# diogoneiss/kubernetes-machine-learning-server

Measured on AMD Instinct MI355X. Metric: itemsets/sec mined (FP-Growth, every frequent itemset of every size + its support, one dataset split over the GPUs), higher is better.
Workload: dtype uint64 tid-bitmaps / exact integer supports

## Files before the change

csrc/emu/kmls/wave.hpp:

```cpp
#pragma once

#include <hip/hip_runtime.h>

#define KMLS_DYN_LDS(T, name) T* name = (T*)emu::dyn_lds()

namespace kmls {
namespace kern {

inline unsigned vzero() { return 0u; }

template <typename T>
using gptr = T*;
template <typename T>
inline gptr<T> as_global(T* p) { return p; }
template <typename T>
inline gptr<T> as_global_addr(unsigned long long a) { return (T*)a; }

inline unsigned long long bcast64(unsigned long long v, int src) {
  return emu::xchg(v, src);
}
inline unsigned long long shfl_xor64(unsigned long long v, int m) {
  return emu::xchg(v, emu::tl->lane ^ m);
}
inline unsigned uni(unsigned v) { return (unsigned)__builtin_amdgcn_readfirstlane((int)v); }
inline unsigned lane0(unsigned v) { return (unsigned)emu::xchg((unsigned long long)v, 0); }
inline unsigned long long lane0_64(unsigned long long v) { return emu::xchg(v, 0); }
inline unsigned long long uni64(unsigned long long v) {
  return ((unsigned long long)uni((unsigned)(v >> 32)) << 32) | uni((unsigned)v);
}

inline unsigned long long ld_agent(const unsigned long long* p) { return __atomic_load_n(p, __ATOMIC_SEQ_CST); }
inline unsigned ld_agent(const unsigned* p) { return __atomic_load_n(p, __ATOMIC_SEQ_CST); }
inline void st_agent(unsigned long long* p, unsigned long long v) { __atomic_store_n(p, v, __ATOMIC_SEQ_CST); }
inline void st_agent(unsigned* p, unsigned v) { __atomic_store_n(p, v, __ATOMIC_SEQ_CST); }
inline void wait_stores() { __atomic_thread_fence(__ATOMIC_SEQ_CST); }
inline void wait_short(unsigned) { std::this_thread::yield(); }

}
}
```

csrc/host/bindings_gpu.cpp:

```cpp
#include <cstring>
#include <pybind11/numpy.h>
#include <pybind11/pybind11.h>
#include <pybind11/stl.h>

#include "../kernels/kernels.hpp"
#include "kmls/gpu.hpp"
#include "kmls/trace.hpp"

namespace py = pybind11;

namespace kmls {

namespace {
template <typename T>
py::array_t<T> to_array(std::vector<T>&& v) {
  auto* heap = new std::vector<T>(std::move(v));
  py::capsule owner(heap, [](void* p) { delete reinterpret_cast<std::vector<T>*>(p); });
  return py::array_t<T>({(py::ssize_t)heap->size()}, {(py::ssize_t)sizeof(T)}, heap->data(), owner);
}

template <typename T>
py::array_t<T> pinned_array(const std::shared_ptr<void>& buf, int64_t n) {
  if (!buf) return py::array_t<T>(0);
  auto* keep = new std::shared_ptr<void>(buf);
// ... 467 lines not shown
        o.assign = assign;
        o.trace = trace;
        o.presplit_cost = presplit_cost;
        o.presplit_budget = presplit_budget;
        o.steal = steal;
        o.steal_idle = steal_idle;
        o.budget0 = budget0;
        o.budget = budget;
        o.split_min = split_min;
        o.blocks_per_cu = blocks_per_cu;
        o.stack_mb = stack_mb;
        gpu::Comm* c = comm.is_none() ? nullptr : comm.cast<gpu::Comm*>();
        gpu::DeepResult r;
        {
          py::gil_scoped_release nogil;
          r = g.mine_deep(ms, max_len, rank, world, c, o);
        }
        py::dict d;
        d["per_level"] = r.per_level;
        d["n_itemsets"] = r.n_itemsets;
        d["n_frequent_items"] = r.n_frequent_items;
        d["max_depth"] = r.max_depth;
        d["candidates"] = r.candidates;
        d["chunks"] = r.chunks;
        d["level2_tasks"] = r.level2_tasks;
        char buf[64];
        std::snprintf(buf, sizeof buf, "%016llx%016llx", (unsigned long long)r.digest_sum,
                      (unsigned long long)r.digest_xor);
        d["digest"] = std::string(buf);
        d["round_tasks"] = r.round_tasks;
        d["spilled_tasks"] = r.spilled_tasks;
        d["handoffs"] = r.handoffs;
        d["leaf_candidates"] = r.leaf_candidates;
        d["leaf_m_default"] = gpu::kDeepLeafDefault;
        d["leaf_m_max"] = kern::deep_leaf_max();
        d["round_ms"] = r.round_ms;
        py::dict ph;
        ph["prologue"] = r.ms_prologue;
        ph["level2_classes"] = r.ms_root;
        ph["rounds"] = r.ms_rounds;
        ph["combine"] = r.ms_combine;
        ph["total"] = r.ms_total;
        ph["assign"] = r.ms_assign;
        ph["presplit"] = r.ms_presplit;
        d["presplit"] = py::make_tuple(r.presplit_in, r.presplit_out);
        if (emit) {
          d["arena_nodes"] = r.arena_nodes;
          d["arena_cap"] = r.arena_cap;
        }
        d["phases_ms"] = ph;
        if (trace) {
          const size_t nw = r.trace.size() / kern::kDeepTraceWords;
          py::array_t<uint64_t> tr({(py::ssize_t)nw, (py::ssize_t)kern::kDeepTraceWords});
          if (!r.trace.empty()) std::memcpy(tr.mutable_data(), r.trace.data(), r.trace.size() * 8);
          d["trace"] = tr;
          d["task_ticks"] = py::array_t<uint64_t>((py::ssize_t)r.task_ticks.size(), r.task_ticks.data());
          d["task_ids"] = py::array_t<int64_t>((py::ssize_t)r.task_ids.size(), r.task_ids.data());
          d["task_cost"] = py::array_t<uint32_t>((py::ssize_t)r.task_cost.size(), r.task_cost.data());
          d["clock_khz"] = r.clock_khz;
          d["t_drain"] = r.t_drain;
          d["trace_bucket"] = r.trace_bucket;
        }
        return d;
      }, py::arg("min_support"), py::arg("max_len") = 0, py::arg("rank") = 0, py::arg("world") = 1,
         py::arg("comm") = py::none(), py::arg("budget0") = 1024ull, py::arg("budget") = 16ull,
         py::arg("split_min") = 8u, py::arg("blocks_per_cu") = 0, py::arg("stack_mb") = 0,
// ... 145 lines not shown
```

csrc/host/deep_gpu.hip:

```cpp
#include <hip/hip_runtime.h>

#include <algorithm>
#include <chrono>
#include <cstring>
#include <stdexcept>
#include <string>
#include <vector>

#include "deep_run.hpp"
#include "kmls/digest.hpp"
#include "kmls/gpu.hpp"

#define KMLS_HIP(expr)                                                                  \
  do {                                                                                  \
    hipError_t _e = (expr);                                                             \
    if (_e != hipSuccess)                                                               \
      throw std::runtime_error(std::string("HIP error ") + hipGetErrorString(_e) +      \
                               " at " + __FILE__ + ":" + std::to_string(__LINE__));     \
  } while (0)

namespace kmls {
namespace gpu {

DeepResult GpuMiner::mine_deep(double min_support, int max_len, int rank, int world, Comm* comm,
// ... 45 lines not shown
  deep_->device = device_;
  DeepInput in;
  in.bm = d_own_bm_;
  in.Wp = Wp;
  in.F = F;
  in.W_real = W_real;
  in.d_ids = d_ids_;
  in.counts = fi_.counts.data();
  in.minsup = minsup;
  in.max_len = max_len;
  in.n_cus = n_cus_;
  in.stream = s;
  res.ms_prologue = ms_since(t0);
  DeepLocal loc;
  for (int attempt = 0;; ++attempt) {
    try {
      loc = deep_run(*deep_, in, rank, world, opt);
      break;
    } catch (const ArenaOverflow& ex) {
      if (attempt >= 2) throw;
    }
  }
  DeepBufs& b = *deep_;
  for (int d = 2; d < 64; ++d) per[(size_t)d] += loc.per_depth[(size_t)d];
  dsum += loc.dsum;
  dxor ^= loc.dxor;
  uint64_t cands = loc.candidates;
  res.chunks = (int64_t)loc.chunks;
  res.level2_tasks = loc.level2_tasks;
  res.round_tasks = loc.round_tasks;
  res.spilled_tasks = loc.spilled_tasks;
  res.handoffs = loc.handoffs;
  res.leaf_candidates = (int64_t)loc.leaf_candidates;
  res.round_ms = loc.round_ms;
  res.ms_root = loc.ms_root;
  res.ms_rounds = loc.ms_rounds;
  res.ms_assign = loc.ms_assign;
  res.ms_presplit = loc.ms_presplit;
  res.arena_nodes = loc.arena_nodes;
  res.arena_cap = deep_->arena_cap;
  res.presplit_in = loc.presplit_in;
  res.presplit_out = loc.presplit_out;
  res.trace = std::move(loc.trace);
  res.task_ticks = std::move(loc.task_ticks);
  res.task_ids = std::move(loc.task_ids);
  res.task_cost = std::move(loc.task_cost);
  res.clock_khz = loc.clock_khz;
  res.t_drain = loc.t_drain;
  res.trace_bucket = loc.trace_bucket;
  if (b.xor_cap < world) {
    if (b.d_xor) KMLS_HIP(hipFree(b.d_xor));
    KMLS_HIP(hipMalloc((void**)&b.d_xor, (size_t)world * 8));
    b.xor_cap = world;
  }

  const auto t3 = now();
  if (comm && world > 1) {
    std::vector<uint64_t> red(66);
    std::copy(per.begin(), per.end(), red.begin());
    red[64] = dsum;
    red[65] = cands;
    KMLS_HIP(hipMemcpyAsync(b.d_red, red.data(), 66 * 8, hipMemcpyHostToDevice, s));
    KMLS_HIP(hipMemcpyAsync(b.d_xor + rank, &dxor, 8, hipMemcpyHostToDevice, s));
    comm->all_reduce(b.d_red, b.d_red, 66, CommDtype::U64, false, s);
    comm->all_gather(b.d_xor + rank, b.d_xor, 1, CommDtype::U64, s);
    std::vector<uint64_t> xs((size_t)world);
// ... 191 lines not shown
```

csrc/host/deep_run.hip:

```cpp
#include "deep_run.hpp"
#include "kmls/hooks.hpp"

#include <algorithm>
#include <chrono>
#include <cstdio>
#include <cstdlib>
#include <stdexcept>
#include <string>

#define KMLS_HIP(expr)                                                                  \
  do {                                                                                  \
    hipError_t _e = (expr);                                                             \
    if (_e != hipSuccess)                                                               \
      throw std::runtime_error(std::string("HIP error ") + hipGetErrorString(_e) +      \
                               " at " + __FILE__ + ":" + std::to_string(__LINE__));     \
  } while (0)

namespace kmls {
namespace gpu {

DeepBufs::~DeepBufs() {
  (void)hipSetDevice(device);
  for (void* p : {(void*)stacks, (void*)stacks0, (void*)fstacks, (void*)q[0], (void*)q[1], (void*)ready, (void*)req, (void*)inbox, (void*)inbox_state, (void*)d_key, (void*)heap[0],
                  (void*)heap[1], (void*)root, (void*)ctl, (void*)d_red, (void*)d_xor,
// ... 481 lines not shown
    KMLS_HIP(hipMemcpyAsync(b.h_ctl, b.ctl, sizeof(kern::DeepCtl), hipMemcpyDeviceToHost, s));
    KMLS_HIP(hipStreamSynchronize(s));
    if (b.h_ctl->error & 4)
      throw std::runtime_error("deep_run: round " + std::to_string(round) +
                               " ran past KMLS_DEEP_ROUND_TIMEOUT_S and gave up");
    if (b.h_ctl->error)
      throw std::runtime_error("deep_run: round " + std::to_string(round) + " failed (" +
                               ((b.h_ctl->error & 8) ? "bad block width" :
                                (b.h_ctl->error & 1) ? "task queue overflow" : "spill heap overflow") +
                               "); raise KMLS_DEEP_QUEUE_MB / KMLS_DEEP_HEAP_MB");
    res.round_tasks.push_back(n_in);
    res.round_ms.push_back(ms_since(tr));
    n_in = (int64_t)b.h_ctl->n_out;
    res.spilled_tasks += n_in;
    cur ^= 1;
  }
  KMLS_HIP(hipMemcpyAsync(b.h_ctl, b.ctl, sizeof(kern::DeepCtl), hipMemcpyDeviceToHost, s));
  KMLS_HIP(hipStreamSynchronize(s));
  res.ms_rounds = ms_since(t2);
  for (int d = 3; d < 64; ++d) res.per_depth[(size_t)d] += b.h_ctl->per_depth[d];
  if (E) {
    const int64_t used = (int64_t)b.h_ctl->node_top;
    b.arena_used = used;
    b.max_depth = 2;
    for (int d = 3; d < 64; ++d)
      if (b.h_ctl->per_depth[d]) b.max_depth = d;
    if (used > b.arena_cap) throw ArenaOverflow(used);
    res.arena_nodes = used;
  }
  res.dsum = b.h_ctl->digest_sum;
  res.dxor = b.h_ctl->digest_xor;
  res.candidates = b.h_ctl->candidates;
  res.leaf_candidates = b.h_ctl->leaf_candidates;
  res.chunks = b.h_ctl->chunks;
  return res;
}

}
}
```

csrc/host/deep_run.hpp:

```cpp
#pragma once

#include <hip/hip_runtime.h>

#include <cstdint>
#include <stdexcept>
#include <vector>

#include "../kernels/kernels.hpp"
#include "kmls/gpu.hpp"

namespace kmls {
namespace gpu {

struct DeepBufs {
  int device = 0;
  char* stacks = nullptr;
  size_t stack_bytes = 0;
  char* stacks0 = nullptr;
  size_t seg0 = 0;
  int64_t waves = 0;
  kern::DeepFrame* fstacks = nullptr;
  int fcap = 0;
  kern::DeepFrame* q[2] = {nullptr, nullptr};
  int64_t q_cap = 0;
// ... 45 lines not shown
  bool t_item16 = true;
  bool t_whole = false;
  int64_t* d_split_q = nullptr;
  int64_t* d_split_heap = nullptr;
  int64_t split_cap = 0;
  int64_t node_off_cap = 0;
  unsigned long long* d_trace = nullptr;
  unsigned long long* d_ticks = nullptr;
  int64_t trace_cap = 0, ticks_cap = 0;
  kern::DeepCtl* ctl = nullptr;
  kern::DeepCtl* h_ctl = nullptr;
  uint64_t* d_red = nullptr;
  uint64_t* d_xor = nullptr;
  int xor_cap = 0;
  ~DeepBufs();
};

struct DeepInput {
  const uint64_t* bm = nullptr;
  int64_t Wp = 0, F = 0;
  int W_real = 0;
  const int32_t* d_ids = nullptr;
  const uint32_t* counts = nullptr;
  uint32_t minsup = 0;
  int max_len = 0;
  int n_cus = 256;
  hipStream_t stream = nullptr;
};

struct DeepLocal {
  std::vector<uint64_t> per_depth = std::vector<uint64_t>(64, 0);
  uint64_t dsum = 0, dxor = 0, candidates = 0, chunks = 0;
  uint64_t leaf_candidates = 0;
  int64_t level2_tasks = 0;
  int maxt = 0;
  std::vector<int64_t> round_tasks;
  int64_t spilled_tasks = 0;
  int64_t handoffs = 0;
  std::vector<double> round_ms;
  double ms_alloc = 0, ms_root = 0, ms_rounds = 0, ms_assign = 0, ms_presplit = 0;
  int64_t presplit_in = 0, presplit_out = 0;
  int64_t arena_nodes = 0;
  std::vector<uint64_t> trace, task_ticks;
  std::vector<int64_t> task_ids;
  std::vector<uint32_t> task_cost;
  double clock_khz = 0;
  uint64_t t_drain = 0, trace_bucket = 0;
};

struct ArenaOverflow : std::runtime_error {
  int64_t needed;
  explicit ArenaOverflow(int64_t n)
      : std::runtime_error("deep_run: node arena overflow"), needed(n) {}
};
DeepLocal deep_run(DeepBufs& b, const DeepInput& in, int rank, int world, const DeepOpts& opt);

}
}
```

csrc/include/kmls/gpu.hpp:

```cpp
#pragma once

#include <cstdint>
#include <memory>
#include <atomic>
#include <mutex>
#include <stdexcept>
#include <string>
#include <utility>
#include <vector>

#include "kmls/comm_host.hpp"
#include "kmls/common.hpp"
#include "kmls/host.hpp"

namespace pybind11 { class module_; }

namespace kmls {

void register_gpu_bindings(pybind11::module_& m);
void register_front_bindings(pybind11::module_& m);

namespace gpu {

bool available();
// ... 96 lines not shown
};

struct OutBufs;
struct DeepBufs;
struct DeepBufsDeleter {
  void operator()(DeepBufs* p) const;
};

struct DeepOpts {
  unsigned long long budget0 = 1024;
  unsigned long long budget = 16;
  unsigned split_min = 8;
  int blocks_per_cu = 0;
  int stack_mb = 0;
  bool steal = true;
  unsigned steal_idle = 1;
  int assign = 1;
  bool trace = false;
  int deal_key = -1;
  unsigned presplit_cost = 16;
  unsigned long long presplit_budget = 1;
  bool emit = false;
};
constexpr int kDeepLeafDefault = 7;
struct DeepResult {
  std::vector<uint64_t> per_level;
  int64_t n_itemsets = 0, n_frequent_items = 0, candidates = 0, chunks = 0, level2_tasks = 0;
  int max_depth = 0;
  uint64_t digest_sum = 0, digest_xor = 0;
  std::vector<int64_t> round_tasks;
  int64_t spilled_tasks = 0;
  int64_t handoffs = 0;
  int64_t leaf_candidates = 0;
  std::vector<double> round_ms;
  double ms_prologue = 0, ms_root = 0, ms_rounds = 0, ms_combine = 0, ms_total = 0;
  double ms_assign = 0;
  int64_t presplit_in = 0, presplit_out = 0;
  double ms_presplit = 0;
  int64_t arena_nodes = 0;
  int64_t arena_cap = 0;
  std::vector<uint64_t> trace, task_ticks;
  std::vector<int64_t> task_ids;
  std::vector<uint32_t> task_cost;
  double clock_khz = 0;
  uint64_t t_drain = 0, trace_bucket = 0;
};
struct GraphCache;
struct Prefetch;
}
namespace kern { struct FCtl; }
namespace gpu {

class GpuMiner {
 public:
  GpuMiner(int device, size_t arena_bytes, uintptr_t stream);
  ~GpuMiner();

  void load_csr(const int64_t* tx_ptr, const int32_t* items, int64_t n_tx, int64_t n_items);
  int64_t n_tx() const { return n_tx_; }
  int64_t n_items() const { return n_items_; }

  void item_support(uintptr_t counts_dev);
  int64_t select(const uint32_t* global_counts, int64_t global_n_tx, double min_support);
  int64_t select_device(const uint32_t* d_counts, int64_t global_n_tx, double min_support,
                        Comm* comm = nullptr);
  void use_frequent_subset(const int64_t* keep, int64_t n);
// ... 247 lines not shown
```

csrc/include/kmls/wave.hpp:

```cpp
#pragma once

#include <hip/hip_runtime.h>

#define KMLS_DYN_LDS(T, name) extern __shared__ T name[]

namespace kmls {
namespace kern {

__device__ __forceinline__ unsigned vzero() {
  unsigned z = 0;
  asm volatile("" : "+v"(z));
  return z;
}

template <typename T>
using gptr = __attribute__((address_space(1))) T*;
template <typename T>
__device__ __forceinline__ gptr<T> as_global(T* p) {
  return (gptr<T>)p;
}
template <typename T>
__device__ __forceinline__ gptr<T> as_global_addr(unsigned long long a) {
  return (gptr<T>)a;
}

__device__ __forceinline__ unsigned long long bcast64(unsigned long long v, int src) {
  const unsigned lo = __shfl((unsigned)v, src, 64);
  const unsigned hi = __shfl((unsigned)(v >> 32), src, 64);
  return ((unsigned long long)hi << 32) | lo;
}

__device__ __forceinline__ unsigned long long shfl_xor64(unsigned long long v, int m) {
  const unsigned lo = __shfl_xor((unsigned)v, m, 64);
  const unsigned hi = __shfl_xor((unsigned)(v >> 32), m, 64);
  return ((unsigned long long)hi << 32) | lo;
}

__device__ __forceinline__ unsigned lane0(unsigned v) {
  return (unsigned)__builtin_amdgcn_readlane((int)v, 0);
}
__device__ __forceinline__ unsigned long long lane0_64(unsigned long long v) {
  return ((unsigned long long)lane0((unsigned)(v >> 32)) << 32) | lane0((unsigned)v);
}

__device__ __forceinline__ unsigned uni(unsigned v) {
  return (unsigned)__builtin_amdgcn_readfirstlane((int)v);
// ... 27 lines not shown
```

csrc/kernels/deep.hip:

```cpp
#include <hip/hip_runtime.h>

#include <algorithm>
#include <cstdint>
#include <type_traits>

#include "kernels.hpp"
#include "kmls/digest.hpp"
#include <kmls/wave.hpp>

namespace kmls {
namespace kern {

namespace {

constexpr int kWaves = 4;
constexpr int kRootChunk = 256;
constexpr int kCap = 512;
constexpr int kBatchFrames = 64;
constexpr int kBStack = 96;
static_assert(kBStack < 127, "block-stack index + 1 must fit the 7 meta bits");
constexpr unsigned kSingle = 1u << 6;
constexpr unsigned kMaxLead = 2047;
constexpr unsigned kDone = 1u << 31;
constexpr unsigned kNodeChunk = 4096;
// ... 162 lines not shown
                                           unsigned long long ih) {
  unsigned long long acc = 0;
  unsigned fill = 0, q = 0;
  const unsigned z = vzero();
#pragma unroll
  for (int w = 0; w < WT; ++w) {
    const unsigned n = uni(P.n[w + z]);
    if (n == 0) continue;
    unsigned long long x = v[w];
#pragma unroll
    for (int i = 0; i < 6; ++i) {
      const unsigned long long t = x & P.mv[i][w + z];
      x = (x ^ t) | (t >> (1u << i));
    }
    acc |= x << fill;
    if (fill + n >= 64) {
      if (surv) cb[(unsigned long long)q * cpad + pos] = acc;
      ++q;
      acc = fill ? (x >> (64 - fill)) : 0ull;
      fill = fill + n - 64;
    } else {
      fill += n;
    }
  }
  if (fill) {
    if (surv) cb[(unsigned long long)q * cpad + pos] = acc;
    ++q;
  }
  for (; q < wt_out; ++q)
    if (surv) cb[(unsigned long long)q * cpad + pos] = 0ull;
  if (surv) cb[(unsigned long long)wt_out * cpad + pos] = ih;
}

template <int MAXT>
struct WaveLds {
  unsigned long long f_hash[kBatchFrames];
  unsigned f_s0[kBatchFrames], f_m[kBatchFrames], f_meta[kBatchFrames];
  unsigned P[kBatchFrames + 1], G[kBatchFrames + 1];
  union {
    struct {
      unsigned short g_cnt[kCap], g_start[kCap];
      unsigned short g_pos[kCap];
      unsigned short g_fi[kCap];
    };
    unsigned long long leaf_rows[kLeafStage];
  };
  unsigned long long g_flag[kCap / 64];
  unsigned b_base[kBStack];
  unsigned b_live[kBStack];
  unsigned long long depth_cnt[64];
  unsigned long long leaf_cands;
  ProjLds<MAXT> proj;
};

struct WaveState {
  unsigned nf;
  unsigned nb;
  unsigned long long mem_top;
  unsigned long long ncur, nend;
};

__device__ __forceinline__ unsigned long long alloc_nodes(const DeepArgs& a, WaveState& st,
                                                          unsigned n, int lane) {
  if (st.ncur + n > st.nend) {
    const unsigned long long chunk = n > kNodeChunk ? n : kNodeChunk;
    unsigned long long b = 0;
    if (lane == 0) b = atomicAdd(&a.ctl->node_top, chunk);
    b = uni64(bcast64(b, 0));
    st.ncur = b;
    st.nend = b + chunk;
  }
  const unsigned long long r = st.ncur;
  st.ncur += n;
  return r;
}

__device__ __forceinline__ void put_node(const DeepArgs& a, unsigned long long id,
                                         unsigned long long parent, unsigned item, unsigned count,
                                         unsigned depth) {
  if (id < a.node_cap) {
    a.node_parent[id] = (unsigned)parent;
    a.node_item[id] = item;
    a.node_count[id] = count;
    a.node_depth[id] = (unsigned char)depth;
// ... 215 lines not shown
}

template <int WT, int MAXT, bool EMIT>
__device__ __forceinline__ void row_step(const DeepArgs& a, DeepFrame* fst, WaveState& st,
                                         WaveLds<MAXT>& L, DeepFrame top, const WaveStack& stack,
                                         int lane, WaveAcc& acc) {
  const unsigned long long lanelt = (1ull << lane) - 1ull;
  const unsigned m = top.m;
  const unsigned depth = meta_depth(top.meta);
  const bool deeper = a.max_len == 0 || (int)depth + 3 <= a.max_len;
  const unsigned nc = m - 1;
  const unsigned long long cpad = roundup16(nc);
  const gptr<const unsigned long long> blk = as_global_addr<const unsigned long long>(top.blk);
  const gptr<const unsigned long long> ihp = blk + (unsigned long long)WT * top.pad;
  const unsigned ia = top.s0;
  const unsigned long long ih_a = ihp[ia + vzero()];
  const unsigned long long h_a = top.hash + ih_a;
  constexpr unsigned E = EMIT ? 1u : 0u;
  const gptr<const unsigned long long> nwp = ihp + top.pad;
  const unsigned long long node_a = E ? uni64(nwp[ia + vzero()] & kDeepNodeMask) : 0ull;
  unsigned wt_out = WT;
  if (WT > 1 && deeper && nc >= 2) {
    const unsigned s = proj_setup<WT>(L.proj, blk, top.pad, ia, lane);
    wt_out = tier_of((s + 63) / 64);
  }
  const bool proj = wt_out < (unsigned)WT;
  unsigned long long* cb =
      stack_block(stack, st.mem_top, (unsigned long long)(wt_out + 1 + E) * cpad * 8ull);
  unsigned S = 0;
  for (unsigned c0 = 0; c0 < nc; c0 += 64) {
    const bool act = c0 + lane < nc;
    const unsigned jb = act ? ia + 1 + c0 + lane : ia;
    unsigned long long v[WT];
    const unsigned long long ih_ld = ihp[jb];
    const unsigned c = and_count<WT>(blk, top.pad, ia + vzero(), jb, v);
    const bool surv = act && c >= a.minsup;
    const unsigned long long mask = __ballot(surv);
    const unsigned pos = S + (unsigned)__popcll(mask & lanelt);
    unsigned long long ih_b = 0;
    if (surv) {
      ih_b = ih_ld;
      const DigestTerms dt = digest_terms(h_a + ih_b, c);
      acc.dsum += dt.sum;
      acc.dxor ^= dt.xr;
    }
    if (deeper) {
      if (proj) {
        write_proj<WT>(cb, cpad, pos, surv, v, L.proj, wt_out, ih_b);
      } else if (surv) {
        write_row<WT>(cb, cpad, pos, v, ih_b);
      }
    }
    if (E && mask) {
      const unsigned long long nb0 = alloc_nodes(a, st, (unsigned)__popcll(mask), lane);
      if (surv) {
        const unsigned long long id = nb0 + (unsigned long long)__popcll(mask & lanelt);
        const unsigned long long nw_b = nwp[jb];
        put_node(a, id, node_a, (unsigned)(nw_b >> 40), c, depth + 2);
        if (deeper) cb[(unsigned long long)(wt_out + 1) * cpad + pos] = ((nw_b >> 40) << 40) | id;
      }
    }
    S += (unsigned)__popcll(mask);
    ++acc.chunks;
  }
  acc.cands += nc;
  if (lane == 0 && S) L.depth_cnt[depth + 2] += S;
  acc.budget_used += (nc + 63) / 64;
  const unsigned lead = meta_lead(top.meta);
  if ((top.meta & kSingle) || m <= 2 || lead == 1u) {
    release_frame(L, top.meta, lane);
    st.nf -= 1;
  } else {
    top.s0 += 1;
    top.m -= 1;
    if (lead) top.meta = meta_with_lead(top.meta, lead - 1u);
    if (lane == 0) store_frame(fst + st.nf - 1, top);
  }
  if (S >= 2 && deeper) {
    if (lane == 0) {
      L.b_base[st.nb] = (unsigned)st.mem_top;
      L.b_live[st.nb] = 1;
      DeepFrame c;
      c.blk = (unsigned long long)cb;
      c.hash = h_a;
      c.pad = (unsigned)cpad;
      c.s0 = 0;
      c.m = S;
      c.meta = make_meta(depth + 1, false, wt_out, st.nb + 1);
      store_frame(fst + st.nf, c);
    }
    st.nb += 1;
    st.nf += 1;
    st.mem_top += (unsigned long long)(wt_out + 1 + E) * cpad * 8ull;
  }
}

template <int WT, int MAXT, bool EMIT>
// ... 49 lines not shown
    unsigned f = 0;
    for (unsigned step = 32; step; step >>= 1)
      if (f + step < k && L.G[f + step] <= g) f += step;
    const unsigned i = g - L.G[f], fmm = L.f_m[f];
    const unsigned pos = L.P[f] + i * fmm - i * (i + 1) / 2;
    L.g_pos[g] = (unsigned short)pos;
    L.g_fi[g] = (unsigned short)((f << 8) | i);
    atomicOr(&L.g_flag[pos >> 6], 1ull << (pos & 63));
  }
  __builtin_amdgcn_wave_barrier();
  const unsigned long long cpad = roundup16(P);
  cb = stack_block(stack, st.mem_top, (unsigned long long)(WT + 1 + (EMIT ? 1u : 0u)) * cpad * 8ull);
  const gptr<const unsigned long long> bblk = as_global_addr<const unsigned long long>(top.blk);
  const unsigned long long bpad = top.pad;
  const gptr<const unsigned long long> ihp = bblk + (unsigned long long)WT * bpad;
  constexpr unsigned E = EMIT ? 1u : 0u;
  const gptr<const unsigned long long> nwp = ihp + bpad;
  unsigned S = 0, gbase = 0;
  for (unsigned c0 = 0; c0 < P; c0 += 64) {
    const unsigned p = c0 + lane;
    const bool act = p < P;
    const unsigned long long gw = uni64(L.g_flag[(c0 >> 6) + vzero()]);
    const unsigned g = gbase + (unsigned)__popcll(gw & ((2ull << lane) - 1ull)) - 1u;
    unsigned f = 0, i = 0, j = 0;
    if (act) {
      const unsigned fi = L.g_fi[g];
      f = fi >> 8;
      i = fi & 0xffu;
      j = i + 1 + (p - L.g_pos[g]);
    }
    gbase += (unsigned)__popcll(gw);
    const unsigned sa = L.f_s0[f] + i, sb = L.f_s0[f] + (act ? j : i);
    unsigned long long v[WT];
    const unsigned long long ih_la = ihp[sa], ih_lb = ihp[sb];
    const unsigned c = and_count<WT>(bblk, bpad, sa, sb, v);
    const bool surv = act && c >= a.minsup;
    const unsigned long long mask = __ballot(surv);
    const bool head = act && (lane == 0 || ((gw >> lane) & 1ull));
    const unsigned long long hmask = __ballot(head);
    if (surv) {
      const unsigned pos = S + (unsigned)__popcll(mask & lanelt);
      const unsigned long long ih_a = ih_la, ih_b = ih_lb;
      write_row<WT>(cb, cpad, pos, v, ih_b);
      const DigestTerms dt = digest_terms(L.f_hash[f] + ih_a + ih_b, c);
      acc.dsum += dt.sum;
      acc.dxor ^= dt.xr;
    }
    if (E && mask) {
      const unsigned long long nb0 = alloc_nodes(a, st, (unsigned)__popcll(mask), lane);
      if (surv) {
        const unsigned pos = S + (unsigned)__popcll(mask & lanelt);
        const unsigned long long id = nb0 + (unsigned long long)__popcll(mask & lanelt);
        const unsigned long long nw_b = nwp[sb];
        put_node(a, id, nwp[sa] & kDeepNodeMask, (unsigned)(nw_b >> 40), c,
                 meta_depth(top.meta) + 2);
        cb[(unsigned long long)(WT + 1) * cpad + pos] = ((nw_b >> 40) << 40) | id;
      }
    }
    if (head) {
      const unsigned long long after = hmask & ~((2ull << lane) - 1ull);
      const unsigned long long below_end = after ? ((1ull << __builtin_ctzll(after)) - 1ull) : ~0ull;
      const unsigned long long rs = mask & below_end & ~lanelt;
      if (rs) {
        L.g_cnt[g] = (unsigned short)(L.g_cnt[g] + (unsigned)__popcll(rs));
        if (L.g_start[g] == 0xffffu) {
          const unsigned first = (unsigned)__builtin_ctzll(rs);
          L.g_start[g] = (unsigned short)(S + (unsigned)__popcll(mask & ((1ull << first) - 1ull)));
        }
      }
    }
    if (lane == 0 && mask) L.depth_cnt[meta_depth(top.meta) + 2] += (unsigned long long)__popcll(mask);
    S += (unsigned)__popcll(mask);
    ++acc.chunks;
  }
  acc.cands += P;
  acc.budget_used += (P + 63) / 64;
  if ((unsigned)lane < k) {
    const unsigned b = meta_bidx(L.f_meta[lane]);
    if (b) atomicSub(&L.b_live[b - 1], 1u);
  }
  st.nf -= k;
  __builtin_amdgcn_wave_barrier();
  unsigned pushed = 0;
  const unsigned nbi = st.nb;
  for (unsigned g0 = 0; g0 < NG; g0 += 64) {
    const unsigned g = g0 + lane;
    bool mk = false;
    unsigned f = 0;
    if (g < NG) {
      for (unsigned step = 32; step; step >>= 1)
        if (f + step < k && L.G[f + step] <= g) f += step;
      mk = L.g_cnt[g] >= 2 && (a.max_len == 0 || (int)meta_depth(L.f_meta[f]) + 3 <= a.max_len);
    }
    const unsigned long long mask = __ballot(mk);
    if (mk) {
      const unsigned slot = st.nf + pushed + (unsigned)__popcll(mask & lanelt);
      const unsigned i = g - L.G[f];
      const unsigned long long ih_a = ihp[L.f_s0[f] + i];
      DeepFrame c;
      c.blk = (unsigned long long)cb;
      c.hash = L.f_hash[f] + ih_a;
      c.pad = (unsigned)cpad;
      c.s0 = L.g_start[g];
      c.m = L.g_cnt[g];
      c.meta = make_meta(meta_depth(L.f_meta[f]) + 1, false, WT, nbi + 1);
      store_frame(fst + slot, c);
    }
    pushed += (unsigned)__popcll(mask);
  }
  pushed = uni(pushed);
  if (pushed) {
    if (lane == 0) {
      L.b_base[st.nb] = (unsigned)st.mem_top;
      L.b_live[st.nb] = pushed;
    }
    st.nb += 1;
    st.nf += pushed;
    st.mem_top += (unsigned long long)(WT + 1 + E) * cpad * 8ull;
  }
}

template <int WT, int MAXT>
__device__ __forceinline__ void leaf_step(const DeepArgs& a, WaveState& st, WaveLds<MAXT>& L,
                                          const DeepFrame& top, const DeepFrame& lf, int lane,
                                          WaveAcc& acc) {
  static_assert(WT <= kLeafTier, "leaf step tiers");
  constexpr unsigned kStride = (unsigned)kLeafStage / (unsigned)(WT + 1);
  const unsigned depth = meta_depth(top.meta);
  const unsigned fm = lf.m;
  const bool elig = (unsigned)lane < st.nf && lf.blk == top.blk &&
                    ((lf.meta ^ top.meta) & 0x3fffu) == 0u &&
                    meta_lead(lf.meta) == 0u && fm >= 2u && fm <= a.leaf_m;
  const unsigned fc = elig ? (1u << fm) - fm - 1u : 0u;
  unsigned incl = fc, lo = lf.s0, hi = lf.s0 + fm;
  for (int off = 1; off < 64; off <<= 1) {
    const unsigned oi = __shfl_up(incl, off, 64), ol = __shfl_up(lo, off, 64),
                   oh = __shfl_up(hi, off, 64);
    if (lane >= off) {
      incl += oi;
      lo = ol < lo ? ol : lo;
      hi = oh > hi ? oh : hi;
    }
  }
  const unsigned long long eligm = __ballot(elig);
  const unsigned run = eligm == ~0ull ? 64u : (unsigned)__builtin_ctzll(~eligm);
  const unsigned long long okm = __ballot((unsigned)lane < run && incl <= (unsigned)kLeafSlots &&
                                          hi - lo + (unsigned)kLeafMax <= kStride);
  unsigned k = okm == ~0ull ? 64u : (unsigned)__builtin_ctzll(~okm);
  if (k == 0) k = 1;
  k = uni(k);
  const unsigned total = uni(__shfl(incl, (int)k - 1, 64));
  const unsigned smin = uni(__shfl(lo, (int)k - 1, 64));
  const unsigned range = uni(__shfl(hi, (int)k - 1, 64)) - smin;
  unsigned mmax = 2;
#pragma unroll
  for (unsigned i = 3; i <= (unsigned)kLeafMax; ++i)
    if (__ballot((unsigned)lane < k && fm >= i)) mmax = i;
  if (lane < (int)(kCap / 64)) L.g_flag[lane] = 0ull;
  __builtin_amdgcn_wave_barrier();
  if ((unsigned)lane < k) {
    const unsigned base = incl - fc;
    L.f_hash[lane] = lf.hash;
    L.f_s0[lane] = lf.s0 - smin;
    L.f_meta[lane] = lf.meta;
    L.P[lane] = base;
    atomicOr(&L.g_flag[base >> 6], 1ull << (base & 63));
  }
  {
    const gptr<const unsigned long long> blk = as_global_addr<const unsigned long long>(top.blk);
#pragma unroll
    for (int w = 0; w <= WT; ++w) {
      const gptr<const unsigned long long> row = blk + (unsigned long long)w * top.pad + smin;
      for (unsigned j = lane; j < range; j += 64) L.leaf_rows[(unsigned)w * kStride + j] = row[j];
    }
  }
  __builtin_amdgcn_wave_barrier();
  unsigned fbase = 0, dc = 0;
  unsigned long long evaluated = 0;
  for (unsigned c0 = 0; c0 < total; c0 += 64) {
    const unsigned p = c0 + lane;
    const unsigned long long gw = uni64(L.g_flag[(c0 >> 6) + vzero()]);
    const unsigned f = fbase + (unsigned)__popcll(gw & ((2ull << lane) - 1ull)) - 1u;
    fbase += (unsigned)__popcll(gw);
    const unsigned mask = p < total ? leaf_subset(p - L.P[f]) : 3u;
    const unsigned kk = (unsigned)__popc(mask);
    const bool act = p < total && (a.max_len == 0 || (int)(depth + kk) <= a.max_len);
    const unsigned o = L.f_s0[f];
    unsigned long long h = L.f_hash[f];
    unsigned long long v[WT];
#pragma unroll
    for (int w = 0; w < WT; ++w) v[w] = ~0ull;
#pragma unroll kLeafUnroll
    for (unsigned i = 0; i < (unsigned)kLeafMax; ++i) {
      if (i >= mmax) break;
      if ((mask >> i) & 1u) {
#pragma unroll
        for (int w = 0; w < WT; ++w) v[w] &= L.leaf_rows[(unsigned)w * kStride + o + i];
        h += L.leaf_rows[(unsigned)WT * kStride + o + i];
      }
    }
    unsigned c = 0;
#pragma unroll
    for (int w = 0; w < WT; ++w) c += (unsigned)__popcll(v[w]);
    const bool surv = act && c >= a.minsup;
    if (surv) {
      const DigestTerms dt = digest_terms(h, c);
      acc.dsum += dt.sum;
      acc.dxor ^= dt.xr;
    }
#pragma unroll
    for (unsigned q = 2; q <= (unsigned)kLeafMax; ++q) {
      if (q > mmax) break;
      const unsigned n = (unsigned)__popcll(__ballot(surv && kk == q));
      if ((unsigned)lane == q) dc += n;
    }
    evaluated += (unsigned long long)__popcll(__ballot(act));
    ++acc.chunks;
  }
  if ((unsigned)lane >= 2u && (unsigned)lane <= mmax && dc && depth + (unsigned)lane < 64u)
    L.depth_cnt[depth + (unsigned)lane] += dc;
  acc.cands += evaluated;
  if (lane == 0) L.leaf_cands += evaluated;
  acc.budget_used += (total + 63) / 64;
  if ((unsigned)lane < k) {
    const unsigned b = meta_bidx(L.f_meta[lane]);
    if (b) atomicSub(&L.b_live[b - 1], 1u);
  }
  st.nf -= k;
  __builtin_amdgcn_wave_barrier();
}

enum StepKind { kStepBatch = 0, kStepRow = 1, kStepLeaf = 2 };

template <int MAXT, bool EMIT, int T0, int... Ts>
__device__ __forceinline__ void step_tier(unsigned wt, StepKind kind, const DeepArgs& a,
                                          DeepFrame* fst, WaveState& st, WaveLds<MAXT>& L,
                                          const DeepFrame& top, const DeepFrame& lf,
                                          const WaveStack& stack, int lane, WaveAcc& acc) {
  if constexpr (T0 <= MAXT) {
    if (wt == (unsigned)T0) {
      if constexpr (!EMIT && T0 <= kLeafTier) {
        if (kind == kStepLeaf) {
          leaf_step<T0, MAXT>(a, st, L, top, lf, lane, acc);
          return;
        }
      }
      if (kind == kStepRow)
        row_step<T0, MAXT, EMIT>(a, fst, st, L, top, stack, lane, acc);
      else
        batch_step<T0, MAXT, EMIT>(a, fst, st, L, top, lf, stack, lane, acc);
      return;
    }
  }
  if constexpr (sizeof...(Ts) > 0)
    step_tier<MAXT, EMIT, Ts...>(wt, kind, a, fst, st, L, top, lf, stack, lane, acc);
}

template <int MAXT>
constexpr int deep_waves_per_simd() { return MAXT <= 16 ? 4 : 2; }

template <int MAXT, int WPS, bool EMIT>
__global__ __launch_bounds__(256, WPS) __attribute__((amdgpu_waves_per_eu(WPS))) void k_deep_count(DeepArgs a) {
  __shared__ WaveLds<MAXT> lds[kWaves];
  const int lane = threadIdx.x & 63;
  const int wid = (int)uni(threadIdx.x >> 6);
  WaveLds<MAXT>& L = lds[wid];
  const unsigned long long gw = (unsigned long long)blockIdx.x * kWaves + wid;
  DeepFrame* fst = a.fstacks + gw * (unsigned long long)a.fcap;
  const WaveStack stack{a.stacks0 ? a.stacks0 + gw * a.seg0 : nullptr,
                        a.stacks + gw * a.stack_bytes, a.stacks0 ? a.seg0 : 0ull};

  for (int d = lane; d < 64; d += 64) L.depth_cnt[d] = 0;
  if (lane == 0) L.leaf_cands = 0;
  WaveAcc acc{0, 0, 0, 0, 0};
  __builtin_amdgcn_wave_barrier();

  WaveState st{0, 0, 0, 0, 0};
  constexpr unsigned E = EMIT ? 1u : 0u;
  bool failed = false;
  const unsigned long long t_start = wall_clock64();
  auto timed_out = [&]() {
    if (wall_clock64() - t_start <= a.timeout_ticks) return false;
    if (lane == 0) atomicOr(&a.ctl->error, 4u);
    return true;
  };
  const unsigned kOpen = (a.epoch << 2) | 1u, kFilling = (a.epoch << 2) | 2u,
                 kFull = (a.epoch << 2) | 3u, kClosed = a.epoch << 2;
  bool holding = false, inbox_open = false;
  unsigned long long t = 0;
  unsigned long long* tr = a.trace ? a.trace + gw * (unsigned long long)kDeepTraceWords : nullptr;
  unsigned victim = (unsigned)((gw * 7919ull + 1) % (unsigned long long)(a.nwaves > 0 ? a.nwaves : 1));
  while (!failed) {
    if (!holding) {
      if (lane == 0) t = atomicAdd(&a.ctl->next_task, 1ull);
      t = uni64(bcast64(t, 0));
      holding = true;
    }
    DeepFrame tf;
    bool task_from_inbox = false;
    unsigned long long task_ticket = t;
    if (!a.steal) {
      if (t >= (unsigned long long)a.n_in) break;
      tf = load_frame(a.in + t, lane);
      holding = false;
    } else {
      if (tr && lane == 0 && t + 1 == (unsigned long long)a.n_in) a.ctl->t_drain = wall_clock64();
// ... 117 lines not shown
        break;
      }
      if (a.steal && acc.budget_used >= a.budget) {
        acc.budget_used = 0;
        if (a.steal_eager == 1) {
          if (spill_frames<MAXT, EMIT>(a, fst, st, L, lane, true, 1) == 0) {
            free_blocks(L, st);
            if (st.nf == 0) break;
            continue;
          }
        } else if (st.nf >= 2 ||
                   (a.split_keep16 && frame_firsts(top.meta, top.m) >= a.split_firsts)) {
          unsigned long long r = 0;
          if (a.steal_eager == 2) {
            r = (gw ^ 1ull) < (unsigned long long)a.nwaves ? (gw ^ 1ull) + 1ull : 0ull;
          } else if (lane == 0) {
            r = ld_agent(&a.req[gw]);
            if ((r >> 32) == (unsigned long long)a.epoch) st_agent(&a.req[gw], 0ull);
            else r = 0;
          }
          r = uni64(bcast64(r, 0));
          if (r && donate_bottom<MAXT, EMIT>(a, fst, st, L, lane, (unsigned)(r & 0xffffffffull) - 1u,
                                       kOpen, kFilling, kFull)) {
            free_blocks(L, st);
            continue;
          }
        }
      }
      if (wt == 0 || wt > (unsigned)MAXT) {
        if (lane == 0) atomicOr(&a.ctl->error, 8u);
        failed = true;
        break;
      }
      step_tier<MAXT, EMIT, 1, 2, 3, 4, 6, 8, 12, 16, 24, 32, 48, 64>(
          wt, leaf_mode ? kStepLeaf : row_mode ? kStepRow : kStepBatch, a, fst, st, L, top, lf, stack,
          lane, acc);
      free_blocks(L, st);
    }
    if (tr && !failed && lane == 0) {
      const unsigned long long now = wall_clock64();
      if (a.trace_bucket) {
        constexpr unsigned long long kLast = (unsigned long long)(kDeepTraceBuckets - 1);
        unsigned long long x0 = tr_t0 - t_start;
        const unsigned long long x1 = now - t_start;
        while (x0 < x1) {
          const unsigned long long b0 = x0 / a.trace_bucket;
          const unsigned long long bk = b0 < kLast ? b0 : kLast;
          const unsigned long long e =
              bk == kLast ? x1 : ((bk + 1) * a.trace_bucket < x1 ? (bk + 1) * a.trace_bucket : x1);
          tr[6 + bk] += e - x0;
          x0 = e;
        }
      }
      tr[4] += now - tr_t0;
      tr[2] = now;
      tr[5] += (1ull << 32) | (task_from_inbox ? 1ull : 0ull);
      if (a.task_ticks && !task_from_inbox && task_ticket < (unsigned long long)a.n_in)
        a.task_ticks[task_ticket] = now - tr_t0;
    }
    if (a.steal && !failed) {
      unsigned long long left = 0;
      if (lane == 0) left = atomicSub(&a.ctl->pending, 1ull);
      left = uni64(bcast64(left, 0));
      if (left == 1) {
        unsigned long long tail = 0;
        if (lane == 0) tail = (unsigned long long)a.n_in + ld_agent(&a.ctl->n_out);
        tail = uni64(bcast64(tail, 0));
        for (unsigned long long k = lane; k < (unsigned long long)a.nwaves; k += 64)
          if (tail + k < (unsigned long long)a.out_cap)
            atomicExch(&a.ready[tail + k - a.n_in], a.epoch ^ kDone);
      }
    }
  }
  for (int off = 32; off; off >>= 1) {
    acc.dsum += shfl_xor64(acc.dsum, off);
    acc.dxor ^= shfl_xor64(acc.dxor, off);
  }
  __builtin_amdgcn_wave_barrier();
  if (lane == 0) {
    atomicAdd(&a.ctl->digest_sum, acc.dsum);
    atomicXor(&a.ctl->digest_xor, acc.dxor);
    atomicAdd(&a.ctl->candidates, acc.cands);
    atomicAdd(&a.ctl->chunks, acc.chunks);
    if (L.leaf_cands) atomicAdd(&a.ctl->leaf_candidates, L.leaf_cands);
  }
  for (int d = lane; d < 64; d += 64)
    if (L.depth_cnt[d]) atomicAdd(&a.ctl->per_depth[d], L.depth_cnt[d]);
  if (tr && lane == 0) {
    tr[0] = t_start;
    tr[3] = wall_clock64();
  }
}


__global__ void k_deep_transpose(const unsigned long long* bm, long long Wp, long long F, int W,
                                 int W_real, const int32_t* ids, unsigned long long* root,
                                 long long Fpad) {
  const long long e = (long long)blockIdx.x * blockDim.x + threadIdx.x;
  const long long tot = (long long)(W + 1) * Fpad;
  if (e >= tot) return;
  const long long w = e / Fpad, i = e - w * Fpad;
  unsigned long long v = 0;
  if (i < F) v = w == W ? item_mix((unsigned long long)ids[i]) : (w < W_real ? bm[i * Wp + w] : 0ull);
  root[e] = v;
}

template <int WT>
__global__ __launch_bounds__(256) void k_deep_root(const unsigned long long* root, long long Fpad,
                                                   long long F, int maxch, unsigned minsup,
                                                   const int32_t* m_in, int32_t* part,
                                                   const long long* blk_off, char* base,
                                                   DeepCtl* ctl, int fill, DeepNodes nodes,
                                                   const uint32_t* gram) {
  __shared__ ProjLds<WT> projs[kWaves];
  const int lane = threadIdx.x & 63;
  const long long gw = (long long)blockIdx.x * (blockDim.x >> 6) + (threadIdx.x >> 6);
  const long long i = gw / maxch;
// ... 429 lines not shown
```

csrc/kernels/kernels.hpp:

```cpp
#pragma once

#include <hip/hip_runtime.h>

#include <cstdint>
#include <functional>
#include <vector>

namespace kmls {
namespace kern {

struct DeepFrame {
  unsigned long long blk;
  unsigned long long hash;
  unsigned pad;
  unsigned s0;
  unsigned m;
  unsigned meta;
};
static_assert(sizeof(DeepFrame) == 32, "DeepFrame is read as 8 dwords");
struct DeepCtl {
  unsigned long long next_task;
  unsigned long long n_out;
  unsigned long long heap_top;
  unsigned long long pending;
  unsigned long long handoffs;
  unsigned long long node_top;
  unsigned long long digest_sum, digest_xor;
  unsigned long long candidates, chunks;
  unsigned long long per_depth[64];
  unsigned error;
  unsigned pad_[3];
  unsigned long long t_drain;
  unsigned long long leaf_candidates;
};
struct DeepArgs {
  const DeepFrame* in;
  long long n_in;
  DeepFrame* out;
  long long out_cap;
  char* heap;
  unsigned long long heap_cap;
  char* stacks;
  unsigned long long stack_bytes;
  char* stacks0;
  unsigned long long seg0;
  DeepFrame* fstacks;
  int fcap;
  DeepCtl* ctl;
  int W;
  unsigned minsup;
  unsigned long long budget;
  int max_len;
  unsigned leaf_m;
  unsigned split_min;
  unsigned long long timeout_ticks;
  unsigned* ready;
  unsigned long long* req;
  DeepFrame* inbox;
  unsigned* inbox_state;
  long long nwaves;
  unsigned epoch;
  int steal;
  unsigned split_firsts;
  unsigned split_keep16;
  unsigned ask_mask;
  unsigned ask_fanout;
// ... 509 lines not shown
```

Measured before the change: 80.87 billion.

## Make leaf enumeration branch-free and tally depth counts with packed shuffles

For narrow tiers the leaf step now pads each staged row block with identity rows (all-ones bitmap, zero hash) and selects a member row or the identity row by address arithmetic. This replaces the per-lane divergent mask branch with straight-line loads. Per-chunk ballot loops for depth counts become a packed per-lane byte tally reduced with shuffles once at the end, and chunk counting and depth updates move out of the inner loops. It also adds step-kind counters and keep64 scheduling hints on the hash loads. The cost is extra LDS reads of identity rows and more LDS atomics per step.

```diff
diff --git a/csrc/emu/kmls/wave.hpp b/csrc/emu/kmls/wave.hpp
--- a/csrc/emu/kmls/wave.hpp
+++ b/csrc/emu/kmls/wave.hpp
@@ -8,6 +8,7 @@
 namespace kern {
 
 inline unsigned vzero() { return 0u; }
+inline void keep64(unsigned long long&) {}
 
 template <typename T>
 using gptr = T*;
diff --git a/csrc/host/bindings_gpu.cpp b/csrc/host/bindings_gpu.cpp
--- a/csrc/host/bindings_gpu.cpp
+++ b/csrc/host/bindings_gpu.cpp
@@ -523,6 +523,9 @@
         d["spilled_tasks"] = r.spilled_tasks;
         d["handoffs"] = r.handoffs;
         d["leaf_candidates"] = r.leaf_candidates;
+        d["leaf_steps"] = r.leaf_steps;
+        d["batch_steps"] = r.batch_steps;
+        d["row_steps"] = r.row_steps;
         d["leaf_m_default"] = gpu::kDeepLeafDefault;
         d["leaf_m_max"] = kern::deep_leaf_max();
         d["round_ms"] = r.round_ms;
diff --git a/csrc/host/deep_gpu.hip b/csrc/host/deep_gpu.hip
--- a/csrc/host/deep_gpu.hip
+++ b/csrc/host/deep_gpu.hip
@@ -101,6 +101,9 @@
   res.spilled_tasks = loc.spilled_tasks;
   res.handoffs = loc.handoffs;
   res.leaf_candidates = (int64_t)loc.leaf_candidates;
+  res.leaf_steps = (int64_t)loc.leaf_steps;
+  res.batch_steps = (int64_t)loc.batch_steps;
+  res.row_steps = (int64_t)loc.row_steps;
   res.round_ms = loc.round_ms;
   res.ms_root = loc.ms_root;
   res.ms_rounds = loc.ms_rounds;
diff --git a/csrc/host/deep_run.hip b/csrc/host/deep_run.hip
--- a/csrc/host/deep_run.hip
+++ b/csrc/host/deep_run.hip
@@ -537,6 +537,9 @@
   res.dxor = b.h_ctl->digest_xor;
   res.candidates = b.h_ctl->candidates;
   res.leaf_candidates = b.h_ctl->leaf_candidates;
+  res.leaf_steps = b.h_ctl->leaf_steps;
+  res.batch_steps = b.h_ctl->batch_steps;
+  res.row_steps = b.h_ctl->row_steps;
   res.chunks = b.h_ctl->chunks;
   return res;
 }
diff --git a/csrc/host/deep_run.hpp b/csrc/host/deep_run.hpp
--- a/csrc/host/deep_run.hpp
+++ b/csrc/host/deep_run.hpp
@@ -101,6 +101,7 @@
   std::vector<uint64_t> per_depth = std::vector<uint64_t>(64, 0);
   uint64_t dsum = 0, dxor = 0, candidates = 0, chunks = 0;
   uint64_t leaf_candidates = 0;
+  uint64_t leaf_steps = 0, batch_steps = 0, row_steps = 0;
   int64_t level2_tasks = 0;
   int maxt = 0;
   std::vector<int64_t> round_tasks;
diff --git a/csrc/include/kmls/gpu.hpp b/csrc/include/kmls/gpu.hpp
--- a/csrc/include/kmls/gpu.hpp
+++ b/csrc/include/kmls/gpu.hpp
@@ -152,6 +152,7 @@
   int64_t spilled_tasks = 0;
   int64_t handoffs = 0;
   int64_t leaf_candidates = 0;
+  int64_t leaf_steps = 0, batch_steps = 0, row_steps = 0;
   std::vector<double> round_ms;
   double ms_prologue = 0, ms_root = 0, ms_rounds = 0, ms_combine = 0, ms_total = 0;
   double ms_assign = 0;
diff --git a/csrc/include/kmls/wave.hpp b/csrc/include/kmls/wave.hpp
--- a/csrc/include/kmls/wave.hpp
+++ b/csrc/include/kmls/wave.hpp
@@ -12,6 +12,8 @@
   asm volatile("" : "+v"(z));
   return z;
 }
+
+__device__ __forceinline__ void keep64(unsigned long long& v) { asm volatile("" : "+v"(v)); }
 
 template <typename T>
 using gptr = __attribute__((address_space(1))) T*;
diff --git a/csrc/kernels/deep.hip b/csrc/kernels/deep.hip
--- a/csrc/kernels/deep.hip
+++ b/csrc/kernels/deep.hip
@@ -218,6 +218,8 @@
   if (surv) cb[(unsigned long long)wt_out * cpad + pos] = ih;
 }
 
+enum StepKind { kStepBatch = 0, kStepRow = 1, kStepLeaf = 2 };
+
 template <int MAXT>
 struct WaveLds {
   unsigned long long f_hash[kBatchFrames];
@@ -236,6 +238,7 @@
   unsigned b_live[kBStack];
   unsigned long long depth_cnt[64];
   unsigned long long leaf_cands;
+  unsigned n_steps[4];
   ProjLds<MAXT> proj;
 };
 
@@ -517,8 +520,9 @@
     const bool act = c0 + lane < nc;
     const unsigned jb = act ? ia + 1 + c0 + lane : ia;
     unsigned long long v[WT];
-    const unsigned long long ih_ld = ihp[jb];
+    unsigned long long ih_ld = ihp[jb];
     const unsigned c = and_count<WT>(blk, top.pad, ia + vzero(), jb, v);
+    keep64(ih_ld);
     const bool surv = act && c >= a.minsup;
     const unsigned long long mask = __ballot(surv);
     const unsigned pos = S + (unsigned)__popcll(mask & lanelt);
@@ -546,8 +550,8 @@
       }
     }
     S += (unsigned)__popcll(mask);
-    ++acc.chunks;
-  }
+  }
+  acc.chunks += (nc + 63) / 64;
   acc.cands += nc;
   if (lane == 0 && S) L.depth_cnt[depth + 2] += S;
   acc.budget_used += (nc + 63) / 64;
@@ -663,8 +667,10 @@
     gbase += (unsigned)__popcll(gw);
     const unsigned sa = L.f_s0[f] + i, sb = L.f_s0[f] + (act ? j : i);
     unsigned long long v[WT];
-    const unsigned long long ih_la = ihp[sa], ih_lb = ihp[sb];
+    unsigned long long ih_la = ihp[sa], ih_lb = ihp[sb];
     const unsigned c = and_count<WT>(bblk, bpad, sa, sb, v);
+    keep64(ih_la);
+    keep64(ih_lb);
     const bool surv = act && c >= a.minsup;
     const unsigned long long mask = __ballot(surv);
     const bool head = act && (lane == 0 || ((gw >> lane) & 1ull));
@@ -700,10 +706,10 @@
         }
       }
     }
-    if (lane == 0 && mask) L.depth_cnt[meta_depth(top.meta) + 2] += (unsigned long long)__popcll(mask);
     S += (unsigned)__popcll(mask);
-    ++acc.chunks;
-  }
+  }
+  acc.chunks += (P + 63) / 64;
+  if (lane == 0 && S) L.depth_cnt[meta_depth(top.meta) + 2] += S;
   acc.cands += P;
   acc.budget_used += (P + 63) / 64;
   if ((unsigned)lane < k) {
@@ -751,12 +757,18 @@
   }
 }
 
+template <int WT>
+constexpr unsigned leaf_flat() { return WT <= 2 ? 4u : WT <= 4 ? 2u : 0u; }
+
 template <int WT, int MAXT>
 __device__ __forceinline__ void leaf_step(const DeepArgs& a, WaveState& st, WaveLds<MAXT>& L,
                                           const DeepFrame& top, const DeepFrame& lf, int lane,
                                           WaveAcc& acc) {
   static_assert(WT <= kLeafTier, "leaf step tiers");
   constexpr unsigned kStride = (unsigned)kLeafStage / (unsigned)(WT + 1);
+  constexpr unsigned kFlat = leaf_flat<WT>();
+  constexpr unsigned kLead = kFlat ? (unsigned)kLeafMax : 0u;
+  static_assert(kFlat == 0 || kLeafMax % kFlat == 0, "member groups");
   const unsigned depth = meta_depth(top.meta);
   const unsigned fm = lf.m;
   const bool elig = (unsigned)lane < st.nf && lf.blk == top.blk &&
@@ -792,7 +804,7 @@
   if ((unsigned)lane < k) {
     const unsigned base = incl - fc;
     L.f_hash[lane] = lf.hash;
-    L.f_s0[lane] = lf.s0 - smin;
+    L.f_s0[lane] = lf.s0 - smin + kLead;
     L.f_meta[lane] = lf.meta;
     L.P[lane] = base;
     atomicOr(&L.g_flag[base >> 6], 1ull << (base & 63));
@@ -802,32 +814,60 @@
 #pragma unroll
     for (int w = 0; w <= WT; ++w) {
       const gptr<const unsigned long long> row = blk + (unsigned long long)w * top.pad + smin;
-      for (unsigned j = lane; j < range; j += 64) L.leaf_rows[(unsigned)w * kStride + j] = row[j];
+      for (unsigned j = lane; j < range; j += 64)
+        L.leaf_rows[(unsigned)w * kStride + kLead + j] = row[j];
+      if (kFlat && lane < kLeafMax) L.leaf_rows[(unsigned)w * kStride + lane] = w < WT ? ~0ull : 0ull;
     }
   }
   __builtin_amdgcn_wave_barrier();
-  unsigned fbase = 0, dc = 0;
-  unsigned long long evaluated = 0;
+  static_assert(kLeafSlots / 64 * 16 <= 255 && kLeafMax - 2 < 8, "tally fields");
+  const bool capped = a.max_len != 0;
+  const unsigned kk_cap = !capped ? 64u : a.max_len > (int)depth ? (unsigned)a.max_len - depth : 0u;
+  unsigned fbase = 0, ev = 0;
+  unsigned long long tally = 0;
   for (unsigned c0 = 0; c0 < total; c0 += 64) {
     const unsigned p = c0 + lane;
     const unsigned long long gw = uni64(L.g_flag[(c0 >> 6) + vzero()]);
     const unsigned f = fbase + (unsigned)__popcll(gw & ((2ull << lane) - 1ull)) - 1u;
     fbase += (unsigned)__popcll(gw);
-    const unsigned mask = p < total ? leaf_subset(p - L.P[f]) : 3u;
+    const unsigned mask = leaf_subset((p < total ? p : total - 1u) - L.P[f]);
     const unsigned kk = (unsigned)__popc(mask);
-    const bool act = p < total && (a.max_len == 0 || (int)(depth + kk) <= a.max_len);
+    const bool act = p < total && kk <= kk_cap;
     const unsigned o = L.f_s0[f];
     unsigned long long h = L.f_hash[f];
     unsigned long long v[WT];
 #pragma unroll
     for (int w = 0; w < WT; ++w) v[w] = ~0ull;
+    if constexpr (kFlat != 0) {
+      const unsigned o8 = o * 8u;
+#pragma unroll
+      for (unsigned i0 = 0; i0 < (unsigned)kLeafMax; i0 += kFlat) {
+        if (i0 && i0 >= mmax) break;
+        unsigned long long r[kFlat][WT + 1];
+#pragma unroll
+        for (unsigned j = 0; j < kFlat; ++j) {
+          const unsigned sel = (0u - ((mask >> (i0 + j)) & 1u)) & o8;
+          const unsigned long long* mp =
+              (const unsigned long long*)((const char*)&L.leaf_rows[i0 + j] + sel);
+#pragma unroll
+          for (int w = 0; w <= WT; ++w) r[j][w] = mp[(unsigned)w * kStride];
+        }
+#pragma unroll
+        for (unsigned j = 0; j < kFlat; ++j) {
+#pragma unroll
+          for (int w = 0; w < WT; ++w) v[w] &= r[j][w];
+          h += r[j][WT];
+        }
+      }
+    } else {
 #pragma unroll kLeafUnroll
-    for (unsigned i = 0; i < (unsigned)kLeafMax; ++i) {
-      if (i >= mmax) break;
-      if ((mask >> i) & 1u) {
-#pragma unroll
-        for (int w = 0; w < WT; ++w) v[w] &= L.leaf_rows[(unsigned)w * kStride + o + i];
-        h += L.leaf_rows[(unsigned)WT * kStride + o + i];
+      for (unsigned i = 0; i < (unsigned)kLeafMax; ++i) {
+        if (i >= mmax) break;
+        if ((mask >> i) & 1u) {
+#pragma unroll
+          for (int w = 0; w < WT; ++w) v[w] &= L.leaf_rows[(unsigned)w * kStride + o + i];
+          h += L.leaf_rows[(unsigned)WT * kStride + o + i];
+        }
       }
     }
     unsigned c = 0;
@@ -838,18 +878,28 @@
       const DigestTerms dt = digest_terms(h, c);
       acc.dsum += dt.sum;
       acc.dxor ^= dt.xr;
-    }
-#pragma unroll
-    for (unsigned q = 2; q <= (unsigned)kLeafMax; ++q) {
-      if (q > mmax) break;
-      const unsigned n = (unsigned)__popcll(__ballot(surv && kk == q));
-      if ((unsigned)lane == q) dc += n;
-    }
-    evaluated += (unsigned long long)__popcll(__ballot(act));
-    ++acc.chunks;
-  }
-  if ((unsigned)lane >= 2u && (unsigned)lane <= mmax && dc && depth + (unsigned)lane < 64u)
-    L.depth_cnt[depth + (unsigned)lane] += dc;
+      tally += 1ull << ((kk - 2u) * 8u);
+    }
+    ev += act ? 1u : 0u;
+  }
+  acc.chunks += (total + 63) / 64;
+  for (int off = 1; off < 16; off <<= 1) tally += shfl_xor64(tally, off);
+  unsigned long long t_even = tally & 0x00ff00ff00ff00ffull;
+  unsigned long long t_odd = (tally >> 8) & 0x00ff00ff00ff00ffull;
+  for (int off = 16; off < 64; off <<= 1) {
+    t_even += shfl_xor64(t_even, off);
+    t_odd += shfl_xor64(t_odd, off);
+  }
+  if ((unsigned)lane >= 2u && (unsigned)lane <= (unsigned)kLeafMax) {
+    const unsigned q = (unsigned)lane - 2u;
+    const unsigned n = (unsigned)(((q & 1u) ? t_odd : t_even) >> ((q >> 1) * 16u)) & 0xffffu;
+    if (n && depth + (unsigned)lane < 64u) L.depth_cnt[depth + (unsigned)lane] += n;
+  }
+  unsigned long long evaluated = total;
+  if (capped) {
+    for (int off = 32; off; off >>= 1) ev += __shfl_xor(ev, off, 64);
+    evaluated = uni(ev);
+  }
   acc.cands += evaluated;
   if (lane == 0) L.leaf_cands += evaluated;
   acc.budget_used += (total + 63) / 64;
@@ -860,8 +910,6 @@
   st.nf -= k;
   __builtin_amdgcn_wave_barrier();
 }
-
-enum StepKind { kStepBatch = 0, kStepRow = 1, kStepLeaf = 2 };
 
 template <int MAXT, bool EMIT, int T0, int... Ts>
 __device__ __forceinline__ void step_tier(unsigned wt, StepKind kind, const DeepArgs& a,
@@ -903,6 +951,7 @@
 
   for (int d = lane; d < 64; d += 64) L.depth_cnt[d] = 0;
   if (lane == 0) L.leaf_cands = 0;
+  if (lane < 4) L.n_steps[lane] = 0;
   WaveAcc acc{0, 0, 0, 0, 0};
   __builtin_amdgcn_wave_barrier();
 
@@ -1086,9 +1135,10 @@
         failed = true;
         break;
       }
-      step_tier<MAXT, EMIT, 1, 2, 3, 4, 6, 8, 12, 16, 24, 32, 48, 64>(
-          wt, leaf_mode ? kStepLeaf : row_mode ? kStepRow : kStepBatch, a, fst, st, L, top, lf, stack,
-          lane, acc);
+      const StepKind kind = leaf_mode ? kStepLeaf : row_mode ? kStepRow : kStepBatch;
+      if (lane == 0) atomicAdd(&L.n_steps[kind], 1u);
+      step_tier<MAXT, EMIT, 1, 2, 3, 4, 6, 8, 12, 16, 24, 32, 48, 64>(wt, kind, a, fst, st, L, top, lf,
+                                                                      stack, lane, acc);
       free_blocks(L, st);
     }
     if (tr && !failed && lane == 0) {
@@ -1137,6 +1187,9 @@
     atomicAdd(&a.ctl->candidates, acc.cands);
     atomicAdd(&a.ctl->chunks, acc.chunks);
     if (L.leaf_cands) atomicAdd(&a.ctl->leaf_candidates, L.leaf_cands);
+    if (L.n_steps[kStepLeaf]) atomicAdd(&a.ctl->leaf_steps, (unsigned long long)L.n_steps[kStepLeaf]);
+    if (L.n_steps[kStepBatch]) atomicAdd(&a.ctl->batch_steps, (unsigned long long)L.n_steps[kStepBatch]);
+    if (L.n_steps[kStepRow]) atomicAdd(&a.ctl->row_steps, (unsigned long long)L.n_steps[kStepRow]);
   }
   for (int d = lane; d < 64; d += 64)
     if (L.depth_cnt[d]) atomicAdd(&a.ctl->per_depth[d], L.depth_cnt[d]);
diff --git a/csrc/kernels/kernels.hpp b/csrc/kernels/kernels.hpp
--- a/csrc/kernels/kernels.hpp
+++ b/csrc/kernels/kernels.hpp
@@ -32,6 +32,7 @@
   unsigned pad_[3];
   unsigned long long t_drain;
   unsigned long long leaf_candidates;
+  unsigned long long leaf_steps, batch_steps, row_steps;
 };
 struct DeepArgs {
   const DeepFrame* in;
```

After: 93.26 billion, median of 6. 1.15x the previous value.
